# Tyler-Sch/pyruhvro

Hardware: AMD Instinct MI355X
Metric: Avro records/sec -> Arrow (direct decode, input and output resident in HBM) (higher is better)
Workload: dtype u8

## Files before the change

pyruhvro_amd/csrc/engine_device_call.cpp:

```cpp
#include "engine_internal.h"

using namespace rhe;

struct rh_decode_call {
  rh_schema* s;
  const CompiledSchema& cs;
  const uint8_t* d_data;
  const uint64_t* d_offsets;
  uint64_t data_len, n, num_chunks;
  rh_opts opts;
  bool want_stats;
  rh_stats st;
  rh_device_result& r;
  HostProf hp;
  int device = 0;
  hipStream_t stream = nullptr;
  ChunkGeo geo_v;
  const ChunkGeo* geo = nullptr;
  uint32_t k = 1;
  int K = 0, nnodes = 0, nbuf = 0;
  const DeviceProgram* dp = nullptr;
  const SpecKernel* sk = nullptr;
  hipFunction_t size_r = nullptr, emit_r = nullptr;
  uint64_t narrow_rows = 0, tile = 0, bpc64 = 0, payload = 0;
  uint32_t nblocks = 0;
  uint64_t o_null = 0, o_tot = 48, ctrl_bytes = 0;
  uint32_t null_slots = rh::kNullSlots;
  Lease ws, hctrl, dtab, prof_buf;
  std::unique_ptr<CtrlLease> ctrl;
  rh::KParams P;
  uint32_t lds_bytes = 0, emit_lds = 0;
  bool profile = false;
  Events ev;
  std::vector<uint64_t> totals;
  uint64_t n_entries = 0, tab_bytes = 0;
  uint64_t* d_sizes = nullptr;
  uint64_t exact = 0;
  bool child_bitmaps = false, fused = false, timed_size = false;
  bool range_of_host_call = false;
  bool single = false;
  std::vector<uint64_t> caps;
  uint64_t arena_cap = 0, o_tick = 0;
  Lease lookback, hcaps;
  double basis = 0;
  bool settled = false;
  bool async = false;
  DoneEvent done;
  hipEvent_t start_after = nullptr, sized = nullptr;
  bool published = false;
  uint32_t token = 0;
  uint64_t o_flag_h = 0;

  rh_decode_call(rh_schema* s_, const uint8_t* data, const uint64_t* offs, uint64_t dl, uint64_t n_, uint64_t nc, const rh_opts* o,
               bool stats, const ChunkGeo* g, rh_device_result& res)
      : s(s_), cs(*s_->cs), d_data(data), d_offsets(offs), data_len(dl), n(n_), num_chunks(nc), opts(o ? *o : default_opts()),
        want_stats(stats), r(res) {
    std::memset(&st, 0, sizeof st);
    if (g) { geo_v = *g; geo = &geo_v; range_of_host_call = true; }
    opts.devices = nullptr; opts.n_devices = 0; opts.device_stats = nullptr; opts.ready = nullptr; opts.gathered = nullptr;
  }

  Lease arena_lease(uint64_t bytes) {
    r.arena_host = false;
    if ((opts.flags & RH_INTERNAL_HOST_ARENA) && !child_bitmaps && env_long("RUHVRO_HIP_HOST_ARENA", 1, 0, 1) != 0) {
      Block b = pin_pool().try_get(bytes, device);
      if (b.p) {
        r.arena_host = true;
        return Lease(pin_pool(), b);
      }
      pin_pool().prefetch(bytes + bytes / 16, device, pinned_budget_left());
    }
    return Lease(dev_pool(), bytes, device);
  }

  void check_bad(const uint8_t* h) {
    unsigned long long fb = *(const unsigned long long*)h;
    if (!fb) return;
    const uint64_t rec = ~fb;
    uint64_t c = r.sz ? std::min<uint64_t>(rec / r.sz, k - 1) : 0;
    uint64_t b = c * bpc64 + (rec - c * r.sz) / tile;
    rh::ErrInfo ei;
    HIPCHK(hipMemcpy(&ei, P.errinfo + b, sizeof ei, hipMemcpyDeviceToHost));
    throw DecodeError(format_error(ei));
  }

  void layout_host() {
    r.data_bytes = totals;
    for (auto t : totals)
      if (t > 0x7FFFFFFFull) {
        count(RH_CTR_OFFSET32_ERRORS);
        throw DecodeError("offset overflow: a chunk's column exceeds the 2^31-1 limit of 32-bit Arrow offsets");
      }
    if (sk)
      for (int d = 1; d < cs.ndom; d++)
        for (uint32_t c = 0; c < k; c++)
          if (totals[(size_t)(d - 1) * k + c] >= narrow_rows) throw NeedWideIndex();
    r.fill_tables();
    exact = r.output_bytes;
  }

  void launch_tail(bool offsets_done) {
    if (nbuf > 0 && (child_bitmaps || !offsets_done) &&
        rh_launch_init(P.bufptr, d_sizes, dp->desc, (uint32_t)nbuf, k, P.first_bad, stream)) throw HipError("k_init launch failed");
    if (n > 0) {
      emit_lds = lds_bytes;
      if (sk ? launch_module(sk->emit_fn, P, nblocks, (uint32_t)tile, emit_lds, stream, ev.at(3), P.ranged ? nullptr : ev.at(4))
             : (cs.projected ? rh_launch_emit_drop : rh_launch_emit)(&P, emit_lds, stream, ev.at(3), ev.at(4)))
        throw HipError("k_emit launch failed");
      if (P.ranged && launch_module(emit_r, P, nblocks + (P.worklist ? rh::kBigFront : 0u), (uint32_t)tile, emit_lds, stream, nullptr, ev.at(4))) throw HipError("k_emit (ranged) launch failed");
    } else {
      ev.rec(3, stream);
      ev.rec(4, stream);
    }
  }

  void exact_tail() {
    ctrl->b.clean = false;
    published = false;
    layout_host();
    r.arena = arena_lease(r.arena_bytes);
    Lease htab(pin_pool(), tab_bytes, device);
    void** hptr = (void**)htab.ptr();
    uint64_t* hsz = (uint64_t*)(htab.ptr() + (uint64_t)std::max(nbuf, 1) * k * 8);
    for (uint32_t c = 0; c < k; c++)
      for (int b = 0; b < nbuf; b++) {
        hptr[(size_t)c * nbuf + b] = r.arena.ptr() + r.buf_off[(size_t)b * k + c];
        hsz[(size_t)c * nbuf + b] = r.buf_size[(size_t)b * k + c];
      }
    HIPCHK(hipMemcpyAsync(dtab.ptr(), htab.ptr(), tab_bytes, hipMemcpyHostToDevice, stream));
    HIPCHK(hipMemsetAsync(ctrl->ptr() + 8, 0, 8, stream));
    launch_tail(false);
    HIPCHK(hipMemcpyAsync(hctrl.ptr(), ctrl->ptr(), o_tot, hipMemcpyDeviceToHost, stream));
    HIPCHK(hipMemcpyAsync(hctrl.ptr() + o_null, ctrl->ptr() + o_null, ctrl_bytes - o_null, hipMemcpyDeviceToHost, stream));
    HIPCHK(hipStreamSynchronize(stream));
    check_bad(hctrl.ptr());
  }

  bool try_single(bool two_sync, long ratio_hook) {
    const bool on = (opts.flags & RH_SINGLE_PASS) != 0 || env_long("RUHVRO_HIP_SINGLE_PASS", kSinglePassDefault, 0, 1) != 0;
    if (!on || range_of_host_call || (opts.flags & (RH_INTERNAL_TWO_PASS | RH_TWO_PASS)) || !sk || K <= 0 || K > 64 || n == 0 || two_sync ||
        ratio_hook >= 0)
      return false;
    if (n_entries > (1u << 16)) return false;
    if (8ull * K * k > 4ull * K * nblocks) return false;
    hipFunction_t fused_fn = sk->fused_fn.load(std::memory_order_acquire);
    if (!fused_fn) {
      if (sk->fused_dead) return false;
      fused_fn = spec_kernel(s, device, compile_policy(opts.flags & 3, n), false, true).fused_fn.load(std::memory_order_acquire);
      if (!fused_fn) return false;
    }
    std::vector<double> per_row;
    {
      std::lock_guard<std::mutex> g(s->mu);
      if ((int)s->per_row.size() != K) return false;
      if (s->single_cooldown > 0) { s->single_cooldown--; return false; }
      per_row = s->per_row;
    }
    const double slack = (double)env_long("RUHVRO_HIP_SINGLE_SLACK_PERMILLE", 1040, 1, 4000) / 1000.0;
    caps.assign((size_t)K * k, 0);
    for (int kk = 0; kk < K; kk++)
      for (uint32_t c = 0; c < k; c++) {
        const uint64_t rows_c = c == k - 1 ? r.rows_last : r.sz;
        uint64_t cap = (uint64_t)(per_row[(size_t)kk] * (double)rows_c * slack) + (slack >= 1.0 ? 4096 : 0);
        uint64_t lim = 0x7FFFFFFFull;
        if (kk < cs.ndom - 1) lim = std::min<uint64_t>(lim, narrow_rows - 1);
        caps[(size_t)kk * k + c] = std::min(cap, lim);
      }
    {
      uint64_t off = 0;
      for (uint32_t c = 0; c < k; c++)
        for (int b = 0; b < nbuf; b++) {
          const rh::BufDesc& d = cs.bufs[b];
          const uint64_t rows0 = c == k - 1 ? r.rows_last : r.sz;
          const uint64_t rows = d.dom == 0 ? rows0 : caps[(size_t)(d.dom - 1) * k + c];
          off += rh::buf_slot_bytes(rh::buf_bytes(d.kind, rows, d.kind == rh::BK_DATA ? caps[(size_t)d.counter * k + c] : 0, nullptr, (uint32_t)d.counter));
        }
      arena_cap = std::max<uint64_t>(off, kAlign);
    }
    count(RH_CTR_SINGLE_PASS_CALLS);
    count(RH_CTR_FUSED_CALLS);
    single = true; fused = true;
    r.arena = Lease(dev_pool(), arena_cap, device);
    lookback = Lease(dev_pool(), std::max<uint64_t>(8ull * K * nblocks, kAlign), device);
    HIPCHK(hipMemsetAsync(lookback.ptr(), 0, 8ull * K * nblocks, stream));
    hcaps = Lease(pin_pool(), 8ull * K * k, device);
    std::memcpy(hcaps.ptr(), caps.data(), 8ull * K * k);
    uint64_t* d_caps = (uint64_t*)P.blocksum;
    HIPCHK(hipMemcpyAsync(d_caps, hcaps.ptr(), 8ull * K * k, hipMemcpyHostToDevice, stream));
    P.lookback = (unsigned long long*)lookback.ptr();
    P.caps = d_caps;
    rh::LParams LP;
    std::memset(&LP, 0, sizeof LP);
    LP.totals = d_caps; LP.desc = dp->desc; LP.sz = r.sz; LP.rows_last = r.rows_last; LP.n = n; LP.k = k;
    LP.nbuf = nbuf; LP.K = K; LP.ndom = cs.ndom; LP.arena = r.arena.ptr(); LP.capacity = r.arena.b.size;
    LP.bufptr = (void**)dtab.ptr(); LP.bufsize = d_sizes; LP.ctrl = P.first_bad; LP.narrow = 0;
    LP.narrow_rows = narrow_rows;
    if (rh_launch_layout(&LP, stream)) throw HipError("k_layout launch failed");
    if (nbuf > 0 && child_bitmaps && rh_launch_init(P.bufptr, d_sizes, dp->desc, (uint32_t)nbuf, k, P.first_bad, stream))
      throw HipError("k_init launch failed");
    const uint64_t tiles_max = std::max<uint64_t>((r.sz + tile - 1) / tile, (r.rows_last + tile - 1) / tile);
    emit_lds = lds_bytes;
    if (launch_module(fused_fn, P, (uint32_t)(tiles_max * k), (uint32_t)tile, emit_lds, stream, ev.at(3), ev.at(4)))
      throw HipError("k_fused launch failed");
    basis = (double)payload + 64.0 * (double)n;
    void* hdev = nullptr;
    if (hipHostGetDevicePointer(&hdev, hctrl.ptr(), 0) == hipSuccess && hdev) {
      static std::atomic<uint32_t> next_token{0x40000001u};
      token = next_token.fetch_add(1);
      if (token == 0) token = next_token.fetch_add(1);
      o_flag_h = align_up(o_null + 4ull * nnodes * k, 8);
      *(volatile uint32_t*)(hctrl.ptr() + o_flag_h) = 0;
      if (rh_launch_publish(ctrl->ptr(), hdev, (uint32_t)(o_null / 4), (uint32_t)(nnodes * (int)k), (uint32_t)(o_flag_h / 4), token, null_slots, stream))
        throw HipError("k_publish launch failed");
      ctrl->b.clean = true;
      published = true;
    } else {
      (void)hipGetLastError();
      HIPCHK(hipMemcpyAsync(hctrl.ptr(), ctrl->ptr(), ctrl_bytes, hipMemcpyDeviceToHost, stream));
      if (async) done.record(device, stream);
    }
    return true;
  }

  void enqueue() {
    Range rk("ruhvro_hip:decode_device (k_size, k_scan, k_layout, k_init, k_emit)");
    if (opts.device >= 0) { HIPCHK(hipSetDevice(opts.device)); device = opts.device; }
    else HIPCHK(hipGetDevice(&device));
    stream = (hipStream_t)opts.stream;
    if ((uintptr_t)d_data & 15) throw std::invalid_argument("device payload pointer must be 16-byte aligned");

    {
      static std::mutex lds_mu;
      static std::vector<int> lds_done;
      std::lock_guard<std::mutex> g(lds_mu);
      if (std::find(lds_done.begin(), lds_done.end(), device) == lds_done.end()) {
        if (rh_set_max_lds(160 * 1024) != 0) throw HipError("cannot raise the dynamic LDS limit of the decode kernels");
        lds_done.push_back(device);
      }
    }

    r.cs = &cs;
    r.device = device;
    r.n = n;
    if (!geo && opts.chunk_rows) {
      if (num_chunks < 1 || num_chunks > 0xFFFFFFFFull || (num_chunks - 1) > n / opts.chunk_rows ||
          (n > 0 && n == (num_chunks - 1) * opts.chunk_rows && num_chunks > 1))
        throw std::invalid_argument("chunk_rows: the n records do not make num_chunks chunks of chunk_rows rows (the last one takes the rest)");
      geo_v.k = (uint32_t)num_chunks;
      geo_v.sz = opts.chunk_rows;
      geo_v.rows_last = n - (num_chunks - 1) * opts.chunk_rows;
      geo_v.payload_bytes = data_len;
      geo = &geo_v;
    }
    k = geo ? geo->k : rh_clamp_chunks(n, num_chunks);
    r.k = k;
    r.sz = geo ? geo->sz : n / k;
    r.rows_last = geo ? geo->rows_last : n - (uint64_t)(k - 1) * r.sz;
    K = cs.K; nnodes = (int)cs.nodes.size(); nbuf = (int)cs.bufs.size();
    dp = &device_program(s, device);

    const int mode = opts.flags & 3;
    narrow_rows = (uint64_t)env_long("RUHVRO_HIP_NARROW_ROWS",
                                     (long)std::min<uint64_t>(1ull << 28, (1ull << 32) / std::max<uint32_t>(cs.max_row_bytes, 16)), 1, 1l << 28);
    const bool narrow_ok = std::max(r.sz, r.rows_last) < narrow_rows;
    if (mode != RH_KERNEL_GENERIC && n > 0 && narrow_ok) {
      const SpecKernel& k0 = spec_kernel(s, device, compile_policy(mode, n));
      if (k0.ok) sk = &k0;
      else if (mode == RH_KERNEL_SPECIALIZED) throw HipError("specialised kernel unavailable: " + k0.why);
    }
    if (sk) {
      const long force = env_long("RUHVRO_HIP_RANGED", -1, 0, 1);
      const bool want = force == 1 || (force != 0 && (s->ranged_calls.load(std::memory_order_relaxed) > 0 || mode == RH_KERNEL_SPECIALIZED));
      if (want && !sk->ranged_dead) {
// ... 97 lines not shown
    hp.mark("events");

    totals.assign((size_t)K * k, 0);
    n_entries = (uint64_t)k * std::max(nbuf, 0);
    tab_bytes = align_up((uint64_t)std::max(nbuf, 1) * k * 16, kAlign);
    dtab = Lease(dev_pool(), tab_bytes, device);
    d_sizes = (uint64_t*)(dtab.ptr() + (uint64_t)std::max(nbuf, 1) * k * 8);
    P.bufptr = (void* const*)dtab.ptr();
    for (const rh::BufDesc& d : cs.bufs) child_bitmaps = child_bitmaps || (d.kind == rh::BK_BITMAP && d.dom != 0);

    const bool two_sync = env_long("RUHVRO_HIP_TWO_SYNC", 0, 0, 1) != 0;
    const long ratio_hook = env_long("RUHVRO_HIP_ARENA_PERMILLE", -1, 0, 1000000);
    const double ratio = ratio_hook >= 0 ? std::max(1e-9, ratio_hook / 1000.0) : s->arena_ratio.load();
    fused = n > 0 && ratio > 0 && !two_sync && n_entries <= (1u << 16);
    if (start_after) HIPCHK(hipStreamWaitEvent(stream, start_after, 0));
    if (try_single(two_sync, ratio_hook)) return;
    timed_size = n > 0 && size_pass;
    if (timed_size) {
      if (P.worklist) HIPCHK(hipMemsetAsync(P.worklist, 0, 8ull + 8ull * nblocks, stream));

      if (sk ? launch_module(sk->size_fn, P, nblocks, (uint32_t)tile, lds_bytes, stream, ev.at(0), P.ranged ? nullptr : ev.at(1))
             : (cs.projected ? rh_launch_size_drop : rh_launch_size)(&P, lds_bytes, stream, ev.at(0), ev.at(1)))
        throw HipError("k_size launch failed");
      if (P.ranged && launch_module(size_r, P, nblocks + (P.worklist ? rh::kBigFront : 0u), (uint32_t)tile, lds_bytes, stream, nullptr, ev.at(1))) throw HipError("k_size (ranged) launch failed");
      if (sized) HIPCHK(hipEventRecord(sized, stream));
      if (K == 0) {
        P.all_careful = 1;
        ev.rec(5, stream);
        ev.rec(2, stream);
      } else if (!fused && rh_launch_scan(&P, stream, ev.at(5), ev.at(2))) throw HipError("k_scan launch failed");
    } else {
      P.all_careful = 1;
      if (sized) HIPCHK(hipEventRecord(sized, stream));
    }
    static const bool no_trust = env_long("RUHVRO_HIP_NO_TRUST", 0, 0, 1) != 0;
    if (no_trust) P.all_careful = 1;
    hp.mark("size+scan_launch");
    basis = (double)payload + 64.0 * (double)n;
    if (fused) {
      count(RH_CTR_FUSED_CALLS);
      const uint64_t capacity = align_up((uint64_t)(ratio * basis * 1.125) + n_entries * kAlign + (1u << 20), kAlign);
      r.arena = arena_lease(capacity);
      rh::LParams LP;
      std::memset(&LP, 0, sizeof LP);
      LP.totals = P.totals; LP.desc = dp->desc; LP.sz = r.sz; LP.rows_last = r.rows_last; LP.n = n; LP.k = k;
      LP.nbuf = nbuf; LP.K = K; LP.ndom = cs.ndom; LP.arena = r.arena.ptr(); LP.capacity = r.arena.b.size;
      LP.bufptr = (void**)dtab.ptr(); LP.bufsize = d_sizes; LP.ctrl = P.first_bad; LP.narrow = sk ? 1u : 0u;
      LP.narrow_rows = narrow_rows;
      if (timed_size && K == 0 && rh_launch_tile_stats(ctrl->ptr(), P.tileflag, nblocks, stream)) throw HipError("k_tile_stats launch failed");
      if ((timed_size && K > 0) ? rh_launch_scan_layout(&P, &LP, stream, ev.at(5), ev.at(2)) : rh_launch_layout(&LP, stream))
        throw HipError("k_scan / k_layout launch failed");
      launch_tail(true);
      hp.mark("layout+emit_launch");
      void* hdev = nullptr;
      static const bool no_publish = env_long("RUHVRO_HIP_NO_PUBLISH", 0, 0, 1) != 0;
      if (!no_publish && hipHostGetDevicePointer(&hdev, hctrl.ptr(), 0) == hipSuccess && hdev) {
        static std::atomic<uint32_t> next_token{1};
        token = next_token.fetch_add(1);
        if (token == 0) token = next_token.fetch_add(1);
        o_flag_h = align_up(o_null + 4ull * nnodes * k, 8);
        *(volatile uint32_t*)(hctrl.ptr() + o_flag_h) = 0;
        if (rh_launch_publish(ctrl->ptr(), hdev, (uint32_t)(o_null / 4), (uint32_t)(nnodes * (int)k), (uint32_t)(o_flag_h / 4), token, null_slots, stream))
          throw HipError("k_publish launch failed");
        ctrl->b.clean = true;
        published = true;
      } else {
        (void)hipGetLastError();
        HIPCHK(hipMemcpyAsync(hctrl.ptr(), ctrl->ptr(), ctrl_bytes, hipMemcpyDeviceToHost, stream));
        if (async) done.record(device, stream);
      }
      hp.mark("d2h_enqueue");
    }
  }

  void finish() {
    if (settled) return;
    settled = true;
    HIPCHK(hipSetDevice(device));
    if (fused) {
      if (published) {
        volatile uint32_t* flag = (volatile uint32_t*)(hctrl.ptr() + o_flag_h);
        for (uint32_t spins = 0; __atomic_load_n(flag, __ATOMIC_ACQUIRE) != token;) {
          if ((++spins & 0xFFFFu) == 0) {
            const hipError_t q = hipStreamQuery(stream);
            if (q == hipSuccess) {
              if (__atomic_load_n(flag, __ATOMIC_ACQUIRE) != token) throw HipError("rh_k_publish finished without publishing its token");
              break;
            }
            if (q != hipErrorNotReady) throw HipError(std::string("stream failed while waiting for a decode call: ") + hipGetErrorString(q));
          }
#if defined(__x86_64__)
          __builtin_ia32_pause();
#endif
        }
      } else if (done.e) {
        done.wait();
      } else {
        HIPCHK(hipStreamSynchronize(stream));
      }
      hp.mark("sync");
      check_bad(hctrl.ptr());
      const uint32_t lflag = *(const uint32_t*)(hctrl.ptr() + 8);
      if (lflag & rh::LF_NEED_RANGED) {
        ctrl->b.clean = published;
        s->ranged_calls.store(kRangedKeep, std::memory_order_relaxed);
        r.arena.release();
        throw NeedRanged();
      }
      if (published && timed_size && !single) {
        const uint32_t* stw = (const uint32_t*)(hctrl.ptr() + 32);
        count(RH_CTR_TILES, nblocks);
        count(RH_CTR_CAREFUL_TILES, stw[0]); count(RH_CTR_OVER_WINDOW_TILES, stw[1]);
        count(RH_CTR_REWALKED_WAVES, stw[2]); count(RH_CTR_SUBTILED_TILES, stw[3]);
        if (stw[1]) s->ranged_calls.store(kRangedKeep, std::memory_order_relaxed);
        else { uint32_t v = s->ranged_calls.load(std::memory_order_relaxed); if (v) s->ranged_calls.compare_exchange_weak(v, v - 1, std::memory_order_relaxed); }
      }
      if (K > 0) std::memcpy(totals.data(), hctrl.ptr() + o_tot, 8ull * K * k);
      if (single) {
        ctrl->b.clean = published;
        if (lflag) {
          if ((lflag & rh::LF_CAPACITY) && env_long("RUHVRO_HIP_SINGLE_SLACK_PERMILLE", 1040, 1, 4000) >= 1000) {
            std::lock_guard<std::mutex> g(s->mu);
            s->single_backoff = std::min<uint32_t>(1024, std::max<uint32_t>(8, s->single_backoff * 2));
            s->single_cooldown = s->single_backoff;
          }
          count(RH_CTR_SINGLE_PASS_FAILOVERS);
          r.arena.release();
          throw NeedTwoPass();
        }
        r.data_bytes = totals;
        r.layout_bytes = caps;
        r.arena_bytes = arena_cap;
        { std::lock_guard<std::mutex> g(s->mu); s->single_backoff = 0; }
      } else if (lflag & rh::LF_CAPACITY) {
        count(RH_CTR_CAPACITY_RETRIES);
        r.arena.release();
        exact_tail();
// ... 30 lines not shown
        for (uint32_t c = 0; c < k; c++) {
          const uint64_t rows_c = c == k - 1 ? r.rows_last : r.sz;
          if (rows_c) pr[(size_t)kk] = std::max(pr[(size_t)kk], (double)totals[(size_t)kk * k + c] / (double)rows_c);
        }
      std::lock_guard<std::mutex> g(s->mu);
      s->per_row = std::move(pr);
    }
    r.nullcount.assign((size_t)nnodes * k, 0);
    if (published) {
      std::memcpy(r.nullcount.data(), hctrl.ptr() + o_null, 4ull * nnodes * k);
    } else {
      const uint32_t* slots = (const uint32_t*)(hctrl.ptr() + o_null);
      for (size_t e = 0; e < (size_t)nnodes * k; e++) {
        uint32_t sum = 0;
        for (uint32_t sl = 0; sl < null_slots; sl++) sum += slots[e * null_slots + sl];
        r.nullcount[e] = sum;
      }
    }
    hp.mark("host_layout");

    if (profile && sk) {
      unsigned long long hr[64 * 32], h[32] = {0};
      HIPCHK(hipMemcpy(hr, prof_buf.ptr(), sizeof hr, hipMemcpyDeviceToHost));
      for (int r0 = 0; r0 < 64; r0++)
        for (int i = 0; i < 32; i++) h[i] += hr[r0 * 32 + i];
      const double waves = (double)nblocks * 4;
      static const char* names2[] = {"offsets", "stage+barrier", "lane_init", "walk1", "scan", "barrier", "layout", "walk2",
                                     "errors+barrier", "flush"};
      static const char* names1[] = {"ticket+zero+barrier", "offsets+stage+barrier", "size_walk", "wave_scan", "barrier", "lookback(wave0)",
                                     "barrier", "prefix", "emit_walk", "errors+flush"};
      const char* const* names = single ? names1 : names2;
      std::fprintf(stderr, "[ruhvro_hip profile] %s cycles/wave:", single ? "single-pass" : "emit");
      for (int i = 0; i < 10; i++) std::fprintf(stderr, " %s=%.0f", names[i], h[i] / waves);
      std::fprintf(stderr, "\n[ruhvro_hip profile] size cycles/wave: stage+barrier=%.0f init=%.0f walk=%.0f tail=%.0f | kernels ms: size=%.3f emit=%.3f\n",
                   h[16] / waves, h[17] / waves, h[18] / waves, h[19] / waves, ev.ms(0, 1), ev.ms(3, 4));
    }
    if (want_stats) {
      st.records = n;
      st.input_bytes = payload;
      st.output_bytes = exact;
      st.chunks = k;
      st.blocks = nblocks;
      st.size_kernel_ms = (timed_size && !single) ? ev.ms(0, 1) : 0.f;
      st.scan_kernel_ms = (timed_size && !single) ? ev.ms(5, 2) : 0.f;
      st.emit_kernel_ms = n > 0 ? ev.ms(3, 4) : 0.f;
      st.specialized = sk ? 1 : 0;
      st.lds_bytes = emit_lds;
    }
    ws.release(); dtab.release(); hctrl.release(); prof_buf.release(); lookback.release(); hcaps.release(); ctrl.reset();
  }

  void drain() noexcept {
    if (stream || device >= 0) { (void)hipSetDevice(device); (void)hipStreamSynchronize(stream); }
  }
};

rh_device_result::rh_device_result() { std::memset(&st, 0, sizeof st); }
rh_device_result::~rh_device_result() {
  if (pending) {
    pending->drain();
    pending.reset();
  }
  parts.clear();
  if (!join_events.empty()) {
    std::lock_guard<std::mutex> g(DoneEvent::mu());
    auto& v = DoneEvent::idle()[device];
    for (hipEvent_t e : join_events) {
      if (v.size() < 64) v.push_back(e);
      else (void)hipEventDestroy(e);
    }
  }
}


namespace rhe {

typedef rh_decode_call DeviceDecode;

rh_device_result* decode_device_impl1(rh_schema* s, const uint8_t* d_data, const uint64_t* d_offsets, uint64_t data_len,
                                      uint64_t n, uint64_t num_chunks, const rh_opts* opts, rh_stats* stats, const ChunkGeo* geo) {
  auto res = std::make_unique<rh_device_result>();
  auto call = std::make_unique<DeviceDecode>(s, d_data, d_offsets, data_len, n, num_chunks, opts, stats != nullptr, geo, *res);
  const bool async = opts && (opts->flags & RH_ASYNC) && !geo;
  call->async = async;
  try {
    call->enqueue();
    if (async && call->fused) {
      res->pending = std::move(call);
      return res.release();
    }
    call->finish();
  } catch (...) {
    call->drain();
    throw;
  }
  if (stats) {
    const float pack = stats->pack_ms, h2d = stats->h2d_ms, d2h = stats->d2h_ms, tot = stats->total_ms;
    *stats = call->st;
    stats->pack_ms = pack; stats->h2d_ms = h2d; stats->d2h_ms = d2h; stats->total_ms = tot;
  }
  return res.release();
}


void settle(rh_device_result* r);

hipEvent_t pooled_event(int device) {
  hipEvent_t e = nullptr;
// ... 202 lines not shown
```

pyruhvro_amd/csrc/engine_internal.h:

```cpp
#pragma once
#include <hip/hip_runtime_api.h>
#include <dlfcn.h>
#include <pthread.h>

extern "C" hipError_t hipExtModuleLaunchKernel(hipFunction_t f, uint32_t globalWorkSizeX, uint32_t globalWorkSizeY,
                                               uint32_t globalWorkSizeZ, uint32_t localWorkSizeX, uint32_t localWorkSizeY,
                                               uint32_t localWorkSizeZ, size_t sharedMemBytes, hipStream_t hStream,
                                               void** kernelParams, void** extra, hipEvent_t startEvent,
                                               hipEvent_t stopEvent, uint32_t flags);

#include <algorithm>
#include <atomic>
#include <chrono>
#include <cstdio>
#include <cstdlib>
#include <cstring>
#include <functional>
#include <map>
#include <condition_variable>
#include <mutex>
#include <string>
#include <thread>
#include <vector>

// ... 415 lines not shown
};

struct rh_device_encoded {
  int device = 0;
  uint64_t n = 0, sz = 0, rows_last = 0;
  uint32_t k = 1;
  rhe::Lease out;
  uint64_t out_bytes = 0;
  std::vector<uint64_t> ooff;
  std::vector<uint64_t> data_bytes;
  uint64_t exact = 0;
  uint64_t rows(uint32_t c) const { return n == 0 ? 0 : (c == k - 1 ? rows_last : sz); }
};

namespace rhe {

struct Slab {
  std::atomic<int> refs{0};
  void* base = nullptr;
  Block pinned;
  void free_mem() {
    if (pinned.p) {
      pinned_result_bytes().fetch_sub(pinned.size);
      pin_pool().put(pinned);
    } else {
      std::free(base);
    }
    pinned = Block();
    base = nullptr;
  }
  static std::atomic<uint64_t>& pinned_result_bytes() {
    static std::atomic<uint64_t> v{0};
    return v;
  }
};

inline uint64_t pinned_budget_left() {
  static const uint64_t bound = (uint64_t)env_long_early("RUHVRO_HIP_PINNED_RESULT_MB", 4096, 0, 1 << 20) << 20;
  const uint64_t used = Slab::pinned_result_bytes().load();
  return used >= bound ? 0 : bound - used;
}

void export_chunk(const rh_device_result& r, uint32_t c, const uint8_t* base, Slab* slab, ArrowArray* out);
void export_field(const rh::ArrowField& f, ArrowSchema* out);
Slab* slab_from_device(const uint8_t* dptr, uint64_t bytes, int device, hipStream_t stream = nullptr);
int to_host_impl(rh_device_result* r, ArrowArray* out_chunks, hipStream_t stream = nullptr);
void settle(rh_device_result* r);

constexpr long kSinglePassDefault = 0;
constexpr int kPublicFlags = 3 | RH_ASYNC | RH_TWO_PASS | RH_SINGLE_PASS;
constexpr int RH_INTERNAL_HOST_ARENA = 0x200;
constexpr int RH_INTERNAL_TWO_PASS = 0x100;
constexpr long kInternalStreamsDefault = 1;
constexpr long kSplitMinDefault = 1000000;

inline long env_long(const char* name, long dflt, long lo, long hi) {
  const char* e = std::getenv(name);
  if (!e || !*e) return dflt;
  char* end = nullptr;
  const long v = std::strtol(e, &end, 10);
  return (end && *end == 0 && v >= lo && v <= hi) ? v : dflt;
}

struct Events {
  hipEvent_t e[6] = {nullptr, nullptr, nullptr, nullptr, nullptr, nullptr};
  bool on = false;
  int device = 0;
  static std::mutex& mu() { static std::mutex m; return m; }
  static std::map<int, std::vector<hipEvent_t>>& idle() { static auto* v = new std::map<int, std::vector<hipEvent_t>>(); return *v; }
  void init() {
    HIPCHK(hipGetDevice(&device));
    {
      std::lock_guard<std::mutex> g(mu());
      auto& v = idle()[device];
      for (auto& x : e)
        if (!v.empty()) { x = v.back(); v.pop_back(); }
    }
    for (auto& x : e)
      if (!x) HIPCHK(hipEventCreate(&x));
    on = true;
  }
  ~Events() {
    if (!on) return;
    std::lock_guard<std::mutex> g(mu());
    auto& v = idle()[device];
    for (auto& x : e) {
      if (!x) continue;
      if (v.size() < 64) v.push_back(x);
      else (void)hipEventDestroy(x);
    }
  }
  void rec(int i, hipStream_t s) { if (on) HIPCHK(hipEventRecord(e[i], s)); }
  hipEvent_t at(int i) const { return on ? e[i] : nullptr; }
  float ms(int a, int b) {
    float t = 0;
    if (on && hipEventElapsedTime(&t, e[a], e[b]) != hipSuccess) { t = 0; (void)hipGetLastError(); }
    return t;
  }
};

struct DoneEvent {
  hipEvent_t e = nullptr;
  int device = 0;
  static std::mutex& mu() { static std::mutex m; return m; }
  static std::map<int, std::vector<hipEvent_t>>& idle() { static auto* v = new std::map<int, std::vector<hipEvent_t>>(); return *v; }
  void record(int dev, hipStream_t s) {
    device = dev;
    {
      std::lock_guard<std::mutex> g(mu());
      auto& v = idle()[device];
      if (!v.empty()) { e = v.back(); v.pop_back(); }
    }
    if (!e) HIPCHK(hipEventCreateWithFlags(&e, hipEventDisableTiming));
    HIPCHK(hipEventRecord(e, s));
  }
  void wait() { if (e) HIPCHK(hipEventSynchronize(e)); }
  ~DoneEvent() {
    if (!e) return;
    std::lock_guard<std::mutex> g(mu());
    auto& v = idle()[device];
    if (v.size() < 64) v.push_back(e);
    else (void)hipEventDestroy(e);
  }
};

struct ChunkGeo {
  uint64_t sz, rows_last;
  uint32_t k;
  uint64_t payload_bytes;
};

rh_device_result* decode_device_impl1(rh_schema* s, const uint8_t* d_data, const uint64_t* d_offsets, uint64_t data_len,
                                      uint64_t n, uint64_t num_chunks, const rh_opts* opts, rh_stats* stats, const ChunkGeo* geo);
rh_device_result* decode_device_split(rh_schema* s, const uint8_t* d_data, const uint64_t* d_offsets, uint64_t data_len, uint64_t n,
                                      const rh_opts& opts, uint32_t k, uint64_t sz, uint64_t rows_last, unsigned G);
rh_device_result* decode_device_impl(rh_schema* s, const uint8_t* d_data, const uint64_t* d_offsets, uint64_t data_len,
                                     uint64_t n, uint64_t num_chunks, const rh_opts* opts, rh_stats* stats,
                                     const ChunkGeo* geo = nullptr);

template <typename F>
int guarded(char** err, F&& f) {
  try {
    return f();
  } catch (const rh::SchemaError& e) {
    if (err) *err = dup_msg(e.what());
    return RH_ERR_SCHEMA;
  } catch (const DecodeError& e) {
    if (err) *err = dup_msg(e.what());
    return RH_ERR_DECODE;
  } catch (const ValueClassError& e) {
    if (err) *err = dup_msg(e.what());
    return RH_ERR_DECODE;
  } catch (const std::invalid_argument& e) {
    if (err) *err = dup_msg(e.what());
    return RH_ERR_ARGUMENT;
  } catch (const std::exception& e) {
    if (err) *err = dup_msg(e.what());
    return RH_ERR_RUNTIME;
  } catch (...) {
    if (err) *err = dup_msg("internal error: unhandled engine signal");
    return RH_ERR_RUNTIME;
  }
}

void require_device();

struct Source {
  const uint8_t* data = nullptr;
  const uint64_t* offsets = nullptr;
  const uint8_t* const* ptrs = nullptr;
  const uint64_t* lens = nullptr;
  bool slices() const { return ptrs != nullptr || (data == nullptr && offsets == nullptr); }
};

void run_threads(unsigned nt, const std::function<void(unsigned)>& f);
int decode_host_impl(rh_schema* s, const Source& src, uint64_t n, uint64_t num_chunks, const rh_opts* opts,
                     ArrowArray* out_chunks, uint32_t* out_k, rh_stats* stats);
// ... 4 lines not shown
```

pyruhvro_amd/csrc/kernels.hip:

```cpp
#include <hip/hip_runtime.h>
#include <hip/hip_ext.h>
#include <stdint.h>

#define RH_DEEP 1

#include "kernel_common.h"
#include "program.h"
#include "walk.h"
#include "walk_drop.h"

namespace rh {

template <int T>
struct ICtx {
  static constexpr bool kWide = true;
  static constexpr bool kSkip = false;
  static constexpr bool kEnumImm = false;
  static constexpr bool kWaveCtr = true;
  static __device__ __forceinline__ bool enum_sym(int, uint32_t, uint32_t&, uint64_t&) { return false; }
  uint32_t* cnt;
  uint32_t* rem;
  uint32_t* nullcnt;
  const uint64_t* bufs;
  const uint32_t* gb;
// ... 266 lines not shown
    v[0] = wave_sum(t.car); v[1] = wave_sum(t.over); v[2] = wave_sum(t.rew); v[3] = wave_sum(t.sub);
  }
  if (lane == 0) {
#pragma unroll
    for (int j = 0; j < 4; j++) wstat[wave * 4 + j] = v[j];
  }
  __syncthreads();
  if (threadIdx.x == 0 && !refused) {
#pragma unroll
    for (int j = 0; j < 4; j++) {
      const uint32_t sum = wstat[j] + wstat[4 + j] + wstat[8 + j] + wstat[12 + j];
      if (sum) __hip_atomic_fetch_add(ctrl32 + 8 + j, sum, __ATOMIC_RELAXED, __HIP_MEMORY_SCOPE_AGENT);
    }
  }
}

template <uint32_t kScanPer>
__device__ __forceinline__ void scan_segment_n(const KParams& P, uint32_t* wt) {
  const uint32_t tid = threadIdx.x, lane = tid & 63, wave = tid >> 6;
  const uint32_t kk = blockIdx.x % (uint32_t)P.K, ch = blockIdx.x / (uint32_t)P.K;
  const uint32_t b0 = ch * P.bpc;
  const uint32_t b1 = ch == P.k - 1 ? P.nblocks : (ch + 1) * P.bpc;
  const uint32_t* in = P.blocksum + (size_t)kk * P.nblocks;
  uint32_t* out = P.blockbase + (size_t)kk * P.nblocks;
  uint64_t carry = 0;
  for (uint32_t base = b0; base < b1; base += kBlock * kScanPer) {
    const uint32_t i0 = base + tid * kScanPer;
    uint32_t v[kScanPer];
    uint32_t sum = 0;
#pragma unroll
    for (uint32_t j = 0; j < kScanPer; j++) {
      v[j] = i0 + j < b1 ? in[i0 + j] : 0;
      sum += v[j];
    }
    const uint32_t incl = wave_incl_scan(sum, lane);
    if (lane == 63) wt[wave] = incl;
    __syncthreads();
    uint32_t woff = 0;
    for (uint32_t w = 0; w < wave; w++) woff += wt[w];
    const uint32_t round = wt[0] + wt[1] + wt[2] + wt[3];
    uint32_t run = (uint32_t)(carry + woff + (incl - sum));
#pragma unroll
    for (uint32_t j = 0; j < kScanPer; j++) {
      if (i0 + j < b1) out[i0 + j] = run;
      run += v[j];
    }
    carry += round;
    __syncthreads();
  }
  if (tid == 0) P.totals[(size_t)kk * P.k + ch] = carry;
}

__device__ __forceinline__ void scan_segment(const KParams& P, uint32_t* wt) {
  if (P.bpc > 1024u) scan_segment_n<8>(P, wt);
  else scan_segment_n<1>(P, wt);
}

extern "C" __global__ void __launch_bounds__(kBlock) rh_k_scan(KParams P) {
  __shared__ uint32_t wt[4];
  scan_segment(P, wt);
}

__device__ __forceinline__ uint64_t layout_entry(const LParams& L, uint32_t e, uint32_t& flag) {
  const uint32_t c = e / (uint32_t)L.nbuf, b = e - c * (uint32_t)L.nbuf;
  const BufDesc d = L.desc[b];
  const uint64_t rows0 = c == L.k - 1 ? L.rows_last : L.sz;
  const uint64_t rows = d.dom == 0 ? rows0 : L.totals[(size_t)(d.dom - 1) * L.k + c];
  const uint64_t tot = d.kind == BK_DATA ? L.totals[(size_t)d.counter * L.k + c] : 0;
  if (tot > 0x7FFFFFFFull || (d.dom != 0 && rows > 0x7FFFFFFFull)) flag |= LF_OFFSET32;
  if (L.narrow && d.dom != 0 && rows >= L.narrow_rows) flag |= LF_NEED_WIDE;
  return buf_bytes(d.kind, rows, tot, nullptr, (uint32_t)d.counter);
}

__device__ __forceinline__ void layout_body(const LParams& L, uint64_t* run_sum, uint32_t* flags_p) {
  uint32_t& flags = *flags_p;
  const uint32_t tid = threadIdx.x;
  const uint32_t E = L.k * (uint32_t)L.nbuf;
  const uint32_t per = (E + kBlock - 1) / kBlock;
  const uint32_t e0 = tid * per < E ? tid * per : E, e1 = e0 + per < E ? e0 + per : E;
  if (tid == 0) flags = 0;
  __syncthreads();
  uint32_t flag = 0;
  uint64_t mine = 0;
  for (uint32_t e = e0; e < e1; e++) mine += buf_slot_bytes(layout_entry(L, e, flag));
  const uint32_t lane = tid & 63, wave = tid >> 6;
  uint64_t incl = mine;
#pragma unroll
  for (int d = 1; d < 64; d <<= 1) {
    const uint64_t up = __shfl_up(incl, d, 64);
    if ((int)lane >= d) incl += up;
  }
  if (lane == 63) run_sum[wave] = incl;
  if (flag) atomicOr(&flags, flag);
  __syncthreads();
  uint64_t wbase = 0;
  for (uint32_t w = 0; w < wave; w++) wbase += run_sum[w];
  if (tid == kBlock - 1) {
    const uint64_t acc = wbase + incl;
    const uint64_t used = acc < kBufAlign ? kBufAlign : acc;
    uint32_t f = flags | (reinterpret_cast<uint32_t*>(L.ctrl)[2] & (uint32_t)LF_NEED_RANGED);
    if (used > L.capacity) f |= LF_CAPACITY;
    L.ctrl[2] = used;
    reinterpret_cast<uint32_t*>(L.ctrl)[2] = f;
    flags = f;
  }
  __syncthreads();
  if (flags) return;
  uint64_t off = wbase + incl - mine;
  uint32_t dummy = 0;
  for (uint32_t e = e0; e < e1; e++) {
    const uint64_t sz = layout_entry(L, e, dummy);
    L.bufptr[e] = L.arena + off;
    L.bufsize[e] = sz;
    if (L.desc[e % (uint32_t)L.nbuf].kind == BK_OFFSETS) *reinterpret_cast<uint32_t*>(L.arena + off) = 0;
    off += buf_slot_bytes(sz);
  }
}

extern "C" __global__ void __launch_bounds__(kBlock) rh_k_layout(LParams L) {
  __shared__ uint64_t run_sum[kBlock];
  __shared__ uint32_t flags;
  layout_body(L, run_sum, &flags);
}

extern "C" __global__ void __launch_bounds__(kBlock) rh_k_scan_layout(KParams P, LParams L) {
  __shared__ uint64_t run_sum[kBlock];
  __shared__ uint32_t wt[4];
  __shared__ uint32_t flags;
  __shared__ uint32_t last;
  __shared__ uint32_t wstat[16];
  uint32_t* const ctrl32 = reinterpret_cast<uint32_t*>(L.ctrl);
  uint32_t s_lo, s_hi;
  {
    const uint32_t kk = blockIdx.x % (uint32_t)P.K, ch = blockIdx.x / (uint32_t)P.K;
    const uint32_t b0 = ch * P.bpc, b1 = ch == P.k - 1 ? P.nblocks : (ch + 1) * P.bpc;
    s_lo = b0 + (uint32_t)((uint64_t)(b1 - b0) * kk / (uint32_t)P.K);
    s_hi = b0 + (uint32_t)((uint64_t)(b1 - b0) * (kk + 1) / (uint32_t)P.K);
  }
  const uint32_t i0 = s_lo + threadIdx.x;
  const uint32_t f0 = i0 < s_hi ? P.tileflag[i0] : 0u;
  const uint32_t f1 = i0 + kBlock < s_hi ? P.tileflag[i0 + kBlock] : 0u;
  const bool refused = (ctrl32[2] & (uint32_t)LF_NEED_RANGED) != 0;
  scan_segment(P, wt);
  TileStat ts;
  tile_stat_add(ts, f0);
  tile_stat_add(ts, f1);
  tile_stats_rest(ts, P.tileflag, s_lo, s_hi);
  tile_stats_commit(ctrl32, ts, refused, wstat);
  if (threadIdx.x == 0) {
    __builtin_amdgcn_fence(__ATOMIC_RELEASE, "agent");
    uint32_t* ticket = reinterpret_cast<uint32_t*>(L.ctrl) + 3;
    const uint32_t t = __hip_atomic_fetch_add(ticket, 1u, __ATOMIC_RELAXED, __HIP_MEMORY_SCOPE_AGENT);
    last = t == gridDim.x - 1 ? 1u : 0u;
    if (last) __builtin_amdgcn_fence(__ATOMIC_ACQUIRE, "agent");
  }
  __syncthreads();
  if (!last) return;
  layout_body(L, run_sum, &flags);
}

extern "C" __global__ void __launch_bounds__(kBlock) rh_k_tile_stats(uint32_t* ctrl32, const uint32_t* tileflag, uint32_t nflags) {
  __shared__ uint32_t wstat[16];
  const uint32_t lo = (uint32_t)((uint64_t)nflags * blockIdx.x / gridDim.x);
  const uint32_t hi = (uint32_t)((uint64_t)nflags * (blockIdx.x + 1) / gridDim.x);
  const uint32_t i0 = lo + threadIdx.x;
  TileStat ts;
  tile_stat_add(ts, i0 < hi ? tileflag[i0] : 0u);
  tile_stat_add(ts, i0 + kBlock < hi ? tileflag[i0 + kBlock] : 0u);
  tile_stats_rest(ts, tileflag, lo, hi);
  tile_stats_commit(ctrl32, ts, (ctrl32[2] & (uint32_t)LF_NEED_RANGED) != 0, wstat);
}

extern "C" __global__ void __launch_bounds__(kBlock) rh_k_publish(uint32_t* ctrl, uint32_t* host, uint32_t head_words,
                                                                 uint32_t null_entries, uint32_t flag_word, uint32_t token, uint32_t nslots) {
  for (uint32_t i = threadIdx.x; i < head_words; i += kBlock) {
    host[i] = ctrl[i];
    ctrl[i] = 0;
  }
  uint32_t* slots = ctrl + head_words;
  for (uint32_t e = threadIdx.x; e < null_entries; e += kBlock) {
    uint32_t sum = 0;
    if (nslots == (uint32_t)kNullSlots) {
      const v4w* p = reinterpret_cast<const v4w*>(slots + (size_t)e * kNullSlots);
#pragma unroll
      for (int q = 0; q < kNullSlots / 4; q++) { const v4w x = p[q]; sum += x.x + x.y + x.z + x.w; }
    } else {
      for (uint32_t q = 0; q < nslots; q++) sum += slots[(size_t)e * nslots + q];
    }
    host[head_words + e] = sum;
  }
  __syncthreads();
  for (uint32_t i = threadIdx.x; i < null_entries * nslots; i += kBlock) slots[i] = 0;
  __threadfence_system();
  __syncthreads();
  if (threadIdx.x == 0) __hip_atomic_store(host + flag_word, token, __ATOMIC_RELEASE, __HIP_MEMORY_SCOPE_SYSTEM);
}

__device__ __forceinline__ bool call_aborted(const unsigned long long* ctrl) {
  return ctrl[0] != 0 || reinterpret_cast<const uint32_t*>(ctrl)[2] != 0;
}

extern "C" __global__ void __launch_bounds__(kBlock) rh_k_init(void* const* bufptr, const uint64_t* bufsize,
                                                              const BufDesc* desc, uint32_t nbuf, uint32_t k,
                                                              const unsigned long long* ctrl) {
  if (call_aborted(ctrl)) return;
  const uint32_t id = blockIdx.x % nbuf;
  const BufDesc d = desc[id];
  uint8_t* p = reinterpret_cast<uint8_t*>(bufptr[blockIdx.x]);
  const uint64_t sz = bufsize[blockIdx.x];
  if (d.kind == BK_OFFSETS) {
    if (threadIdx.x == 0) *reinterpret_cast<uint32_t*>(p) = 0;
// ... 158 lines not shown
```

Baseline: 9.676 billion.

## Prefetch layout descriptors, widen scan segment unrolls, add optional publish side stream

The scan+layout kernel now loads the first two buffer descriptors and the ranged flag before the scan and ticket wait, so their latency overlaps with scan work. Segment scans gain 16- and 24-wide unrolled variants for large blocks-per-chunk. The publish path is factored into a helper that can run on a separate non-blocking stream, but that option is off by default. The risks are extra register pressure in the scan+layout kernel and a behavioural change in layout_body, which now prefetches descriptors in every block even though only the last block uses them.

```diff
diff --git a/pyruhvro_amd/csrc/engine_device_call.cpp b/pyruhvro_amd/csrc/engine_device_call.cpp
--- a/pyruhvro_amd/csrc/engine_device_call.cpp
+++ b/pyruhvro_amd/csrc/engine_device_call.cpp
@@ -50,6 +50,7 @@
   bool published = false;
   uint32_t token = 0;
   uint64_t o_flag_h = 0;
+  hipStream_t pub_stream = nullptr;
 
   rh_decode_call(rh_schema* s_, const uint8_t* data, const uint64_t* offs, uint64_t dl, uint64_t n_, uint64_t nc, const rh_opts* o,
                bool stats, const ChunkGeo* g, rh_device_result& res)
@@ -134,6 +135,32 @@
     HIPCHK(hipMemcpyAsync(hctrl.ptr() + o_null, ctrl->ptr() + o_null, ctrl_bytes - o_null, hipMemcpyDeviceToHost, stream));
     HIPCHK(hipStreamSynchronize(stream));
     check_bad(hctrl.ptr());
+  }
+
+  void launch_publish(std::atomic<uint32_t>& next_token, bool no_publish) {
+    void* hdev = nullptr;
+    if (!no_publish && hipHostGetDevicePointer(&hdev, hctrl.ptr(), 0) == hipSuccess && hdev) {
+      token = next_token.fetch_add(1);
+      if (token == 0) token = next_token.fetch_add(1);
+      o_flag_h = align_up(o_null + 4ull * nnodes * k, 8);
+      *(volatile uint32_t*)(hctrl.ptr() + o_flag_h) = 0;
+      static const bool side = env_long("RUHVRO_HIP_PUBLISH_STREAM", kPublishStreamDefault, 0, 1) != 0;
+      hipStream_t ps = stream;
+      if (side && async && !range_of_host_call) {
+        ps = publish_stream(device);
+        done.record(device, stream);
+        HIPCHK(hipStreamWaitEvent(ps, done.e, 0));
+        pub_stream = ps;
+      }
+      if (rh_launch_publish(ctrl->ptr(), hdev, (uint32_t)(o_null / 4), (uint32_t)(nnodes * (int)k), (uint32_t)(o_flag_h / 4), token, null_slots, ps))
+        throw HipError("k_publish launch failed");
+      ctrl->b.clean = true;
+      published = true;
+    } else {
+      (void)hipGetLastError();
+      HIPCHK(hipMemcpyAsync(hctrl.ptr(), ctrl->ptr(), ctrl_bytes, hipMemcpyDeviceToHost, stream));
+      if (async) done.record(device, stream);
+    }
   }
 
   bool try_single(bool two_sync, long ratio_hook) {
@@ -203,22 +230,8 @@
     if (launch_module(fused_fn, P, (uint32_t)(tiles_max * k), (uint32_t)tile, emit_lds, stream, ev.at(3), ev.at(4)))
       throw HipError("k_fused launch failed");
     basis = (double)payload + 64.0 * (double)n;
-    void* hdev = nullptr;
-    if (hipHostGetDevicePointer(&hdev, hctrl.ptr(), 0) == hipSuccess && hdev) {
-      static std::atomic<uint32_t> next_token{0x40000001u};
-      token = next_token.fetch_add(1);
-      if (token == 0) token = next_token.fetch_add(1);
-      o_flag_h = align_up(o_null + 4ull * nnodes * k, 8);
-      *(volatile uint32_t*)(hctrl.ptr() + o_flag_h) = 0;
-      if (rh_launch_publish(ctrl->ptr(), hdev, (uint32_t)(o_null / 4), (uint32_t)(nnodes * (int)k), (uint32_t)(o_flag_h / 4), token, null_slots, stream))
-        throw HipError("k_publish launch failed");
-      ctrl->b.clean = true;
-      published = true;
-    } else {
-      (void)hipGetLastError();
-      HIPCHK(hipMemcpyAsync(hctrl.ptr(), ctrl->ptr(), ctrl_bytes, hipMemcpyDeviceToHost, stream));
-      if (async) done.record(device, stream);
-    }
+    static std::atomic<uint32_t> next_token{0x40000001u};
+    launch_publish(next_token, false);
     return true;
   }
 
@@ -422,23 +435,9 @@
         throw HipError("k_scan / k_layout launch failed");
       launch_tail(true);
       hp.mark("layout+emit_launch");
-      void* hdev = nullptr;
       static const bool no_publish = env_long("RUHVRO_HIP_NO_PUBLISH", 0, 0, 1) != 0;
-      if (!no_publish && hipHostGetDevicePointer(&hdev, hctrl.ptr(), 0) == hipSuccess && hdev) {
-        static std::atomic<uint32_t> next_token{1};
-        token = next_token.fetch_add(1);
-        if (token == 0) token = next_token.fetch_add(1);
-        o_flag_h = align_up(o_null + 4ull * nnodes * k, 8);
-        *(volatile uint32_t*)(hctrl.ptr() + o_flag_h) = 0;
-        if (rh_launch_publish(ctrl->ptr(), hdev, (uint32_t)(o_null / 4), (uint32_t)(nnodes * (int)k), (uint32_t)(o_flag_h / 4), token, null_slots, stream))
-          throw HipError("k_publish launch failed");
-        ctrl->b.clean = true;
-        published = true;
-      } else {
-        (void)hipGetLastError();
-        HIPCHK(hipMemcpyAsync(hctrl.ptr(), ctrl->ptr(), ctrl_bytes, hipMemcpyDeviceToHost, stream));
-        if (async) done.record(device, stream);
-      }
+      static std::atomic<uint32_t> next_token{1};
+      launch_publish(next_token, no_publish);
       hp.mark("d2h_enqueue");
     }
   }
@@ -452,7 +451,7 @@
         volatile uint32_t* flag = (volatile uint32_t*)(hctrl.ptr() + o_flag_h);
         for (uint32_t spins = 0; __atomic_load_n(flag, __ATOMIC_ACQUIRE) != token;) {
           if ((++spins & 0xFFFFu) == 0) {
-            const hipError_t q = hipStreamQuery(stream);
+            const hipError_t q = hipStreamQuery(pub_stream ? pub_stream : stream);
             if (q == hipSuccess) {
               if (__atomic_load_n(flag, __ATOMIC_ACQUIRE) != token) throw HipError("rh_k_publish finished without publishing its token");
               break;
@@ -589,8 +588,20 @@
 
   void drain() noexcept {
     if (stream || device >= 0) { (void)hipSetDevice(device); (void)hipStreamSynchronize(stream); }
+    if (pub_stream) (void)hipStreamSynchronize(pub_stream);
   }
 };
+
+namespace rhe {
+hipStream_t publish_stream(int device) {
+  static std::mutex mu;
+  static std::map<int, hipStream_t> all;
+  std::lock_guard<std::mutex> g(mu);
+  hipStream_t& x = all[device];
+  if (!x) HIPCHK(hipStreamCreateWithFlags(&x, hipStreamNonBlocking));
+  return x;
+}
+}
 
 rh_device_result::rh_device_result() { std::memset(&st, 0, sizeof st); }
 rh_device_result::~rh_device_result() {
diff --git a/pyruhvro_amd/csrc/engine_internal.h b/pyruhvro_amd/csrc/engine_internal.h
--- a/pyruhvro_amd/csrc/engine_internal.h
+++ b/pyruhvro_amd/csrc/engine_internal.h
@@ -491,6 +491,7 @@
 constexpr int RH_INTERNAL_HOST_ARENA = 0x200;
 constexpr int RH_INTERNAL_TWO_PASS = 0x100;
 constexpr long kInternalStreamsDefault = 1;
+constexpr long kPublishStreamDefault = 0;
 constexpr long kSplitMinDefault = 1000000;
 
 inline long env_long(const char* name, long dflt, long lo, long hi) {
@@ -562,6 +563,8 @@
     else (void)hipEventDestroy(e);
   }
 };
+
+hipStream_t publish_stream(int device);
 
 struct ChunkGeo {
   uint64_t sz, rows_last;
diff --git a/pyruhvro_amd/csrc/kernels.hip b/pyruhvro_amd/csrc/kernels.hip
--- a/pyruhvro_amd/csrc/kernels.hip
+++ b/pyruhvro_amd/csrc/kernels.hip
@@ -342,8 +342,10 @@
 }
 
 __device__ __forceinline__ void scan_segment(const KParams& P, uint32_t* wt) {
-  if (P.bpc > 1024u) scan_segment_n<8>(P, wt);
-  else scan_segment_n<1>(P, wt);
+  if (P.bpc <= 1024u) scan_segment_n<1>(P, wt);
+  else if (P.bpc <= 8u * kBlock) scan_segment_n<8>(P, wt);
+  else if (P.bpc <= 16u * kBlock) scan_segment_n<16>(P, wt);
+  else scan_segment_n<24>(P, wt);
 }
 
 extern "C" __global__ void __launch_bounds__(kBlock) rh_k_scan(KParams P) {
@@ -351,9 +353,7 @@
   scan_segment(P, wt);
 }
 
-__device__ __forceinline__ uint64_t layout_entry(const LParams& L, uint32_t e, uint32_t& flag) {
-  const uint32_t c = e / (uint32_t)L.nbuf, b = e - c * (uint32_t)L.nbuf;
-  const BufDesc d = L.desc[b];
+__device__ __forceinline__ uint64_t layout_entry(const LParams& L, uint32_t c, const BufDesc& d, uint32_t& flag) {
   const uint64_t rows0 = c == L.k - 1 ? L.rows_last : L.sz;
   const uint64_t rows = d.dom == 0 ? rows0 : L.totals[(size_t)(d.dom - 1) * L.k + c];
   const uint64_t tot = d.kind == BK_DATA ? L.totals[(size_t)d.counter * L.k + c] : 0;
@@ -362,17 +362,48 @@
   return buf_bytes(d.kind, rows, tot, nullptr, (uint32_t)d.counter);
 }
 
-__device__ __forceinline__ void layout_body(const LParams& L, uint64_t* run_sum, uint32_t* flags_p) {
+constexpr uint32_t kLayoutPre = 2;
+struct LayoutPre {
+  BufDesc d[kLayoutPre];
+  uint32_t ranged;
+};
+__device__ __forceinline__ void layout_span(const LParams& L, uint32_t& e0, uint32_t& e1) {
+  const uint32_t E = L.k * (uint32_t)L.nbuf;
+  const uint32_t per = (E + kBlock - 1) / kBlock;
+  e0 = threadIdx.x * per < E ? threadIdx.x * per : E;
+  e1 = e0 + per < E ? e0 + per : E;
+}
+__device__ __forceinline__ void layout_prefetch(const LParams& L, LayoutPre& pre) {
+  uint32_t e0, e1;
+  layout_span(L, e0, e1);
+#pragma unroll
+  for (uint32_t j = 0; j < kLayoutPre; j++) {
+    pre.d[j] = BufDesc{0, 0, 0, 0};
+    if (e0 + j < e1) pre.d[j] = L.desc[(e0 + j) % (uint32_t)L.nbuf];
+  }
+  pre.ranged = reinterpret_cast<const uint32_t*>(L.ctrl)[2] & (uint32_t)LF_NEED_RANGED;
+}
+
+__device__ __forceinline__ void layout_body(const LParams& L, const LayoutPre& pre, uint64_t* run_sum, uint32_t* flags_p) {
   uint32_t& flags = *flags_p;
   const uint32_t tid = threadIdx.x;
-  const uint32_t E = L.k * (uint32_t)L.nbuf;
-  const uint32_t per = (E + kBlock - 1) / kBlock;
-  const uint32_t e0 = tid * per < E ? tid * per : E, e1 = e0 + per < E ? e0 + per : E;
+  uint32_t e0, e1;
+  layout_span(L, e0, e1);
   if (tid == 0) flags = 0;
   __syncthreads();
   uint32_t flag = 0;
   uint64_t mine = 0;
-  for (uint32_t e = e0; e < e1; e++) mine += buf_slot_bytes(layout_entry(L, e, flag));
+  uint64_t szp[kLayoutPre];
+#pragma unroll
+  for (uint32_t j = 0; j < kLayoutPre; j++) {
+    szp[j] = 0;
+    if (e0 + j < e1) {
+      szp[j] = layout_entry(L, (e0 + j) / (uint32_t)L.nbuf, pre.d[j], flag);
+      mine += buf_slot_bytes(szp[j]);
+    }
+  }
+  for (uint32_t e = e0 + kLayoutPre; e < e1; e++)
+    mine += buf_slot_bytes(layout_entry(L, e / (uint32_t)L.nbuf, L.desc[e % (uint32_t)L.nbuf], flag));
   const uint32_t lane = tid & 63, wave = tid >> 6;
   uint64_t incl = mine;
 #pragma unroll
@@ -388,7 +419,7 @@
   if (tid == kBlock - 1) {
     const uint64_t acc = wbase + incl;
     const uint64_t used = acc < kBufAlign ? kBufAlign : acc;
-    uint32_t f = flags | (reinterpret_cast<uint32_t*>(L.ctrl)[2] & (uint32_t)LF_NEED_RANGED);
+    uint32_t f = flags | pre.ranged;
     if (used > L.capacity) f |= LF_CAPACITY;
     L.ctrl[2] = used;
     reinterpret_cast<uint32_t*>(L.ctrl)[2] = f;
@@ -398,19 +429,27 @@
   if (flags) return;
   uint64_t off = wbase + incl - mine;
   uint32_t dummy = 0;
-  for (uint32_t e = e0; e < e1; e++) {
-    const uint64_t sz = layout_entry(L, e, dummy);
+  auto place = [&](uint32_t e, int32_t kind, uint64_t sz) {
     L.bufptr[e] = L.arena + off;
     L.bufsize[e] = sz;
-    if (L.desc[e % (uint32_t)L.nbuf].kind == BK_OFFSETS) *reinterpret_cast<uint32_t*>(L.arena + off) = 0;
+    if (kind == BK_OFFSETS) *reinterpret_cast<uint32_t*>(L.arena + off) = 0;
     off += buf_slot_bytes(sz);
+  };
+#pragma unroll
+  for (uint32_t j = 0; j < kLayoutPre; j++)
+    if (e0 + j < e1) place(e0 + j, pre.d[j].kind, szp[j]);
+  for (uint32_t e = e0 + kLayoutPre; e < e1; e++) {
+    const BufDesc d = L.desc[e % (uint32_t)L.nbuf];
+    place(e, d.kind, layout_entry(L, e / (uint32_t)L.nbuf, d, dummy));
   }
 }
 
 extern "C" __global__ void __launch_bounds__(kBlock) rh_k_layout(LParams L) {
   __shared__ uint64_t run_sum[kBlock];
   __shared__ uint32_t flags;
-  layout_body(L, run_sum, &flags);
+  LayoutPre pre;
+  layout_prefetch(L, pre);
+  layout_body(L, pre, run_sum, &flags);
 }
 
 extern "C" __global__ void __launch_bounds__(kBlock) rh_k_scan_layout(KParams P, LParams L) {
@@ -430,7 +469,9 @@
   const uint32_t i0 = s_lo + threadIdx.x;
   const uint32_t f0 = i0 < s_hi ? P.tileflag[i0] : 0u;
   const uint32_t f1 = i0 + kBlock < s_hi ? P.tileflag[i0 + kBlock] : 0u;
-  const bool refused = (ctrl32[2] & (uint32_t)LF_NEED_RANGED) != 0;
+  LayoutPre pre;
+  layout_prefetch(L, pre);
+  const bool refused = pre.ranged != 0;
   scan_segment(P, wt);
   TileStat ts;
   tile_stat_add(ts, f0);
@@ -446,7 +487,7 @@
   }
   __syncthreads();
   if (!last) return;
-  layout_body(L, run_sum, &flags);
+  layout_body(L, pre, run_sum, &flags);
 }
 
 extern "C" __global__ void __launch_bounds__(kBlock) rh_k_tile_stats(uint32_t* ctrl32, const uint32_t* tileflag, uint32_t nflags) {
```

Measured after the change: 9.675 billion. Within noise of the previous version (-0.0%).
